# robertknight/ocrs-models

Hardware: AMD Instinct MI355X
Metric: detection train-step images/sec (higher is better)
Workload: dtype bf16

## Files before the change

### include/ocrs_hip.h

```cpp
#ifndef OCRS_HIP_H
#define OCRS_HIP_H

#ifdef __cplusplus
extern "C" {
#endif

#ifndef __HIP_PLATFORM_AMD__
typedef struct ihipStream_t* hipStream_t;
#endif

int ocrs_pack_frags(const float* src, int mode, int K, int M, int K2, long s1, long s2, long sm, void* out, int dtype, hipStream_t st);
long ocrs_pack_frags_bytes(int K, int M, int dtype);
int ocrs_pack_frags_multi(const long long* table, int n, long max_frag_threads, int dtype, hipStream_t st);

int ocrs_dwpw_fwd(const void* xa, const void* xb, int Ca, int Cb, const float* tra, const float* trb, const float* wdw, const void* wpk,
                  void* z, double* gstat, const float* gamma, void* pooled, int Cout, int N, int H, int W, int dtype, hipStream_t st);
long ocrs_dwpw_fwd_fin_supported(int Cin, int Cout, int dtype);
int ocrs_dwpw_fwd_fin(const void* xa, const void* xb, int Ca, int Cb, const float* tra, const float* trb, const float* wdw, const void* wpk, void* z,
                      double* gstat, unsigned* counter, long count, const float* bn_w, const float* bn_b, float eps, float momentum, float* tr, float* saved,
                      float* run_mean, float* run_var, long long* nbt, float lo, int Cout, int N, int H, int W, int dtype, hipStream_t st);
long ocrs_dwpw_fwd_pool_supported(int Cin, int Cout);
long ocrs_rs32_fwd_supported(int Ca, int Cb, int Cout, int dtype);
int ocrs_rs32_fwd(const float* xa, const float* xb, int Ca, int Cb, const float* tra, const float* trb, const float* wdw, const float* wpw, float* z,
                  double* gstat, const float* gamma, float* pooled, unsigned* counter, long count, const float* bn_w, const float* bn_b, float eps,
                  float momentum, float* tr, float* saved, float* run_mean, float* run_var, long long* nbt, float lo, int Cout, int N, int H, int W,
                  hipStream_t st);
long ocrs_rs32_bwd_supported(int Ca, int Cb, int Cout, int pooled, int dtype);
long ocrs_rs32_bwd_ws_floats(int Ca, int Cb, int Cout, int N, int H, int W);
int ocrs_rs32_bwd(const float* xa, const float* xb, int Ca, int Cb, const float* tra, const float* trb, const float* wdw, const float* wpw, const float* g1,
                  const float* g2, const float* z, const float* bn, const double* gsum, const float* gamma, const float* saved, float* dgamma, float* dbeta,
                  float* gxa, float* gxb, float* dwpw, float* dwdw, float* ws, const float* saved_a, double* gsum_a, const float* saved_b, double* gsum_b,
                  int pooled, int Cout, int N, int H, int W, hipStream_t st);
long ocrs_rs32_bwd_head_supported(int Ca, int Cb, int Cout, int dtype);
int ocrs_rs32_bwd_head(const float* xa, int Ca, const float* tra, const float* wdw, const float* wpw, const float* gl, const float* whead, const float* z,
                       const float* bn, const double* gsum, const float* gamma, const float* saved, float* dgamma, float* dbeta, float* gxa, float* dwpw,
                       float* dwdw, float* ws, const float* saved_a, double* gsum_a, int Cout, int N, int H, int W, hipStream_t st);
long ocrs_mm_fwd_supported(int Ca, int Cb, int Cout, int dtype);
long ocrs_mm_fwd_nparts(int Ca, int Cb, int Cout, int N, int H, int W);
int ocrs_mm_fwd(const void* xa, const void* xb, int Ca, int Cb, const float* tra, const float* trb, const float* wdw, const float* wpw, void* z,
                float* ws, const float* gamma, void* pooled, int Cout, int N, int H, int W, int dtype, hipStream_t st);
int ocrs_mm_fwd_fin(const void* xa, const void* xb, int Ca, int Cb, const float* tra, const float* trb, const float* wdw, const float* wpw, void* z, float* ws,
                    const float* gamma, void* pooled, unsigned* counter, long count, const float* bn_w, const float* bn_b, float eps, float momentum, float* tr,
                    float* saved, float* run_mean, float* run_var, long long* nbt, float lo, int Cout, int N, int H, int W, int dtype, hipStream_t st);
int ocrs_mm_fwd_fin_xu(const void* xu, const float* wexp, const float* tra, const float* wdw, const float* wpw, void* z, float* ws, unsigned* counter, long count,
                       const float* bn_w, const float* bn_b, float eps, float momentum, float* tr, float* saved, float* run_mean, float* run_var, long long* nbt,
                       float lo, int Cout, int N, int H, int W, int dtype, hipStream_t st);
int ocrs_bn_finalize_parts(const float* parts, int nparts, long count, int C, const float* gamma, const float* beta, float eps, float momentum,
                           float* tr, float* saved, float* run_mean, float* run_var, long long* nbt, float lo, hipStream_t st);
int ocrs_dwpw_c1_fwd(const float* img, const float* wdw, const float* wpw, void* z, double* gstat, int N, int H, int W, int dtype,
                     hipStream_t st);
long ocrs_dwpw_c1_u_supported(int N, int H, int W, int dtype);
int ocrs_dwpw_c1_fwd_u(const float* img, const float* wdw, const float* wpw, void* z, void* uplane, double* gstat, int N, int H, int W, int dtype,
                       hipStream_t st);
int ocrs_bn_finalize(const double* gstat, long count, int C, const float* gamma, const float* beta, float eps, float momentum, float* tr,
                     float* saved, float* run_mean, float* run_var, long long* nbt, float lo, hipStream_t st);
int ocrs_maxpool_fwd(const void* z, const float* tr, void* out, int C, int N, int H, int W, int raw, int dtype, hipStream_t st);
int ocrs_convt_fwd(const void* x, const float* tr, const void* wpk, const float* bias, void* out, int Cup, int Cout, int N, int h, int w,
                   int H, int W, int dtype, hipStream_t st);
long ocrs_rs32_convt_fwd_supported(int Cup, int Cout, int dtype);
int ocrs_rs32_convt_fwd(const float* x, const float* tr, const float* wt, const float* bias, float* out, int Cup, int Cout, int N, int h, int w, int H, int W,
                        hipStream_t st);
long ocrs_rs32_convt_dgrad_supported(int Cup, int Cout, int dtype);
int ocrs_rs32_convt_dgrad(const float* g, const float* wt, float* dx, const float* x, const float* tr, const float* saved, double* gsum, int Cup, int Cout, int N,
                          int h, int w, int H, int W, hipStream_t st);
int ocrs_head_fwd(const void* z, const float* tr, const float* w, const float* b, float* pred, long P, int dtype, hipStream_t st);

int ocrs_bn_bwd_reduce(const void* g1, const void* g2, int pooled, const void* z, const float* bn, const float* saved, double* gsum, int C,
                       int N, int H, int W, int dtype, hipStream_t st);
int ocrs_bn_bwd_finalize(const double* gsum, long count, int C, const float* gamma, const float* saved, float* coef, float* dgamma,
                         float* dbeta, hipStream_t st);
long ocrs_pw_bwd_ws_floats(int Cin, int Cout, int N, int H, int W);
int ocrs_pw_bwd(const void* xa, const void* xb, int Ca, int Cb, const float* tra, const float* trb, const float* wdw, const void* g1,
                const void* g2, int pooled, const void* z, const float* bn, const float* coef, const void* wpk_d, void* du, float* dwpw,
                float* ws, int Cout, int N, int H, int W, int dtype, hipStream_t st);
int ocrs_pw_bwd_fin(const void* xa, const void* xb, int Ca, int Cb, const float* tra, const float* trb, const float* wdw, const void* g1, const void* g2,
                    int pooled, const void* z, const float* bn, float* coef, const double* gsum, const float* gamma, const float* saved, float* dgamma,
                    float* dbeta, const void* wpk_d, void* du, float* dwpw, float* ws, int Cout, int N, int H, int W, int dtype, hipStream_t st);
long ocrs_dw_bwd_ws_floats(int C, int N, int H, int W);
int ocrs_dw_bwd(const void* xa, const void* xb, int Ca, int Cb, const float* tra, const float* trb, const float* wdw, const void* du,
                void* gxa, void* gxb, float* dwdw, float* ws, const float* saved_a, double* gsum_a, const float* saved_b, double* gsum_b,
                int N, int H, int W, int dtype, hipStream_t st);
long ocrs_mm_bwd_supported(int Ca, int Cb, int Cout, int dtype);
long ocrs_mm_bwd_ws_floats(int Ca, int Cb, int Cout, int N, int H, int W);
int ocrs_mm_bwd(const void* xa, const void* xb, int Ca, int Cb, const float* tra, const float* trb, const float* wdw, const float* wpw,
                const void* g1, const void* g2, int pooled, const void* z, const float* bn, const float* coef, void* gxa, void* gxb, float* dwpw,
                float* dwdw, float* ws, const float* saved_a, double* gsum_a, const float* saved_b, double* gsum_b, int Cout, int N, int H,
                int W, int dtype, hipStream_t st);
int ocrs_mm_bwd_fin(const void* xa, const void* xb, int Ca, int Cb, const float* tra, const float* trb, const float* wdw, const float* wpw, const void* g1,
                    const void* g2, int pooled, const void* z, const float* bn, const double* gsum, const float* gamma, const float* saved, float* dgamma,
                    float* dbeta, void* gxa, void* gxb, float* dwpw, float* dwdw, float* ws, const float* saved_a, double* gsum_a, const float* saved_b,
                    double* gsum_b, int Cout, int N, int H, int W, int dtype, hipStream_t st);
long ocrs_mm_bwd_head_supported(int Ca, int Cb, int Cout, int N, int H, int W, int dtype);
int ocrs_mm_bwd_fin_head(const void* xa, int Ca, const float* tra, const float* wdw, const float* wpw, const float* gl, const float* whead, const void* z,
                         const float* bn, const double* gsum, const float* gamma, const float* saved, float* dgamma, float* dbeta, void* gxa, float* dwpw,
                         float* dwdw, float* ws, const float* saved_a, double* gsum_a, int Cout, int N, int H, int W, int dtype, hipStream_t st);
int ocrs_mm_bwd_fin_xu(const void* xu, const float* wexp, const float* tra, const float* wdw, const float* wpw, const void* g1, const void* g2, const void* z,
                       const float* bn, const double* gsum, const float* gamma, const float* saved, float* dgamma, float* dbeta, void* gxa, float* dwpw,
                       float* dwdw, float* ws, const float* saved_a, double* gsum_a, int Cout, int N, int H, int W, int dtype, hipStream_t st);
int ocrs_dwpw_c1_bwd(const float* img, const float* wdw, const float* wpw, const void* g1, const void* g2, int pooled, const void* z,
                     const float* bn, const float* coef, double* acc64, int N, int H, int W, int dtype, hipStream_t st);
long ocrs_convt_bwd_ws_floats(int Cup, int Cout, int N, int h, int w, int dtype);
int ocrs_convt_bwd(const void* x, const float* tr, const void* g, const void* wpk_d, void* dx, float* dW, float* dbias, double* dbias64, float* ws,
// ... 213 lines not shown
```

### ocrs_models_amd/csrc/det_dwf.hip

```cpp
#include "det_common.h"

namespace {
template <int CIN, int COUT>
struct DwfCfg {
    static constexpr int NT = 512, NW = 8;
    static constexpr int TW = 8, TH = (CIN >= 128 || COUT > 128) ? 4 : 8, TP = TW * TH, NNT = TP / 16, HWp = TW + 2, HP = HWp * (TH + 2);
    static constexpr int CGI = CIN / 8;
    static constexpr int PXC = CIN + 8;
    static constexpr int NXI = (HP * CGI + NT - 1) / NT;
    static constexpr int NUI = (TP * CGI + NT - 1) / NT;
    static constexpr int MTO = COUT / 16, NKD = CIN / 32;
    static constexpr int MPW = MTO >= NW ? MTO / NW : 1;
    static constexpr int NPW = MTO >= NW ? NNT : NNT * MTO / NW;
    static constexpr int OFF_U = HP * PXC * 2, OFF_PAR = (OFF_U + TP * PXC * 2 + 15) & ~15;
    static constexpr int SMEM = OFF_PAR + (3 * CIN + 9 * CIN + NW * 2 * COUT) * 4;
    static_assert(NT % CGI == 0 && NPW >= 1 && MTO >= 4, "role mapping");
};
__device__ __forceinline__ void unpack8w(const uint4& r, float (&v)[8]) {
    v[0] = __uint_as_float(r.x << 16); v[1] = __uint_as_float(r.x & 0xffff0000u);
    v[2] = __uint_as_float(r.y << 16); v[3] = __uint_as_float(r.y & 0xffff0000u);
    v[4] = __uint_as_float(r.z << 16); v[5] = __uint_as_float(r.z & 0xffff0000u);
    v[6] = __uint_as_float(r.w << 16); v[7] = __uint_as_float(r.w & 0xffff0000u);
}
}

template <int CIN, int COUT>
__global__ __launch_bounds__(512) void k_dwf(Src2<bf16> x, const float* __restrict__ tra, const float* __restrict__ trb, const float* __restrict__ wdw,
                                             const void* __restrict__ wpk, bf16* __restrict__ z, double* __restrict__ gstat, Tiling2 tg, FwdFin fin) {
    using C = DwfCfg<CIN, COUT>;
    constexpr int NT = C::NT, TW = C::TW, TP = C::TP, HWp = C::HWp, HP = C::HP, CGI = C::CGI, PXC = C::PXC;
    constexpr int NXI = C::NXI, NUI = C::NUI, MTO = C::MTO, NKD = C::NKD, MPW = C::MPW, NPW = C::NPW;
    extern __shared__ __attribute__((aligned(16))) char smem[];
    bf16* xs = reinterpret_cast<bf16*>(smem);
    bf16* uN = reinterpret_cast<bf16*>(smem + C::OFF_U);
    float* s_trx = reinterpret_cast<float*>(smem + C::OFF_PAR);
    float* s_wdw = s_trx + 3 * CIN;
    float* s_st = s_wdw + 9 * CIN;
    const int H = tg.H, W = tg.W;
    const int tid = threadIdx.x, lane = tid & 63, wave = __builtin_amdgcn_readfirstlane(tid >> 6);
    fill_tr8(s_trx, x, tra, trb, CIN, tid);
    for (int i = tid; i < 9 * CIN; i += NT) {
        const int t = i / CIN, c = i - t * CIN;
        s_wdw[i] = wdw[c * 9 + t];
    }
    {
        const uint4 z4 = make_uint4(0, 0, 0, 0);
        for (int i = tid; i < C::OFF_PAR / 16; i += NT) reinterpret_cast<uint4*>(smem)[i] = z4;
    }
    __syncthreads();

    const int cgi = tid % CGI;
    const int m0w = MTO >= C::NW ? wave * MPW : wave % MTO, n0w = MTO >= C::NW ? 0 : (wave / MTO) * NPW;
    Mma<bf16>::Frag wf[NKD][MPW];
#pragma unroll
    for (int kc = 0; kc < NKD; ++kc)
#pragma unroll
        for (int a = 0; a < MPW; ++a) wf[kc][a] = Mma<bf16>::load_w(wpk, (long)kc * MTO + m0w + a, lane);
    float s1[MPW][4], s2[MPW][4];
#pragma unroll
    for (int a = 0; a < MPW; ++a)
#pragma unroll
        for (int i = 0; i < 4; ++i) s1[a][i] = s2[a][i] = 0.f;

    struct Raw {
        uint4 xr[NXI];
        unsigned okx;
    };
    auto issue = [&](Raw& r, const TileOrg& org) {
        r.okx = 0;
        const int c0 = cgi * 8;
        const bool from_a = c0 < x.Ca;
        const bf16* xb = from_a ? x.a + c0 : x.b + (c0 - x.Ca);
        const int pitch = from_a ? x.Ca : x.Cb;
        const long corner = ((long)org.n * H + (org.h0 - 1)) * W + (org.w0 - 1);
#pragma unroll
        for (int j = 0; j < NXI; ++j) {
            const int hp = (tid + j * NT) / CGI, hy = hp / HWp, hx = hp - hy * HWp;
            const int h = org.h0 - 1 + hy, w = org.w0 - 1 + hx;
            const bool ok = (HP * CGI % NT == 0 || tid + j * NT < HP * CGI) && (unsigned)h < (unsigned)H && (unsigned)w < (unsigned)W;
            r.xr[j] = *reinterpret_cast<const uint4*>(ok ? xb + (corner + (long)hy * W + hx) * pitch : xb);
            r.okx |= ok ? 1u << j : 0u;
        }
    };
    auto commit = [&](const Raw& r) {
        float sc[8], sh[8], lo[8];
        load8(s_trx + cgi * 24, sc);
        load8(s_trx + cgi * 24 + 8, sh);
        load8(s_trx + cgi * 24 + 16, lo);
#pragma unroll
        for (int j = 0; j < NXI; ++j) {
            if (HP * CGI % NT != 0 && tid + j * NT >= HP * CGI) break;
            float v[8] = {0.f, 0.f, 0.f, 0.f, 0.f, 0.f, 0.f, 0.f};
            if (r.okx & (1u << j)) {
                unpack8w(r.xr[j], v);
#pragma unroll
                for (int i = 0; i < 8; ++i) v[i] = max_lo(fmaf(v[i], sc[i], sh[i]), lo[i]);
            }
            store8_opaque(xs + ((tid + j * NT) / CGI) * PXC + cgi * 8, v);
            __builtin_amdgcn_sched_barrier(0);
        }
    };

    TileSched ts(tg.ntiles);
    Raw cur;
    if (ts.first < ts.end) issue(cur, tile_origin2<TW, C::TH>(tg, (int)ts.first));
    for (long t = ts.first; t < ts.end; t += ts.step) {
        const TileOrg org = tile_origin2<TW, C::TH>(tg, (int)t);
        commit(cur);
        __syncthreads();
        if (t + ts.step < ts.end) issue(cur, tile_origin2<TW, C::TH>(tg, (int)(t + ts.step)));
        {
            float u[NUI][8];
#pragma unroll
            for (int j = 0; j < NUI; ++j)
#pragma unroll
                for (int i = 0; i < 8; ++i) u[j][i] = 0.f;
#pragma unroll
            for (int tap = 0; tap < 9; ++tap) {
                float wv[8];
                load8(s_wdw + tap * CIN + cgi * 8, wv);
#pragma unroll
                for (int j = 0; j < NUI; ++j) {
                    const int pxl = (tid + j * NT) / CGI, ty = pxl / TW, tx = pxl - ty * TW;
                    if (TP * CGI % NT == 0 || tid + j * NT < TP * CGI) {
                        float v[8];
                        unpack8w(*reinterpret_cast<const uint4*>(xs + ((ty + tap / 3) * HWp + tx + tap % 3) * PXC + cgi * 8), v);
#pragma unroll
                        for (int i = 0; i < 8; ++i) u[j][i] = fmaf(wv[i], v[i], u[j][i]);
                    }
                }
                if (tap % 3 == 2) __builtin_amdgcn_sched_barrier(0);
            }
#pragma unroll
            for (int j = 0; j < NUI; ++j)
                if (TP * CGI % NT == 0 || tid + j * NT < TP * CGI) store8_opaque(uN + ((tid + j * NT) / CGI) * PXC + cgi * 8, u[j]);
        }
        __syncthreads();
        {
            f32x4 acc[MPW][NPW];
#pragma unroll
            for (int a = 0; a < MPW; ++a)
#pragma unroll
                for (int b = 0; b < NPW; ++b) acc[a][b] = (f32x4){0.f, 0.f, 0.f, 0.f};
#pragma unroll
            for (int kc = 0; kc < NKD; ++kc)
#pragma unroll
                for (int b = 0; b < NPW; ++b) {
                    const Mma<bf16>::Frag pf = Mma<bf16>::load_p(uN + kc * 32, PXC, (n0w + b) * 16, lane, 32);
#pragma unroll
                    for (int a = 0; a < MPW; ++a) acc[a][b] = Mma<bf16>::template mma<8>(wf[kc][a], pf, acc[a][b]);
                }
#pragma unroll
            for (int b = 0; b < NPW; ++b) {
                const int oq = (n0w + b) * 16 + (lane & 15);
                const int qh = org.h0 + oq / TW, qw = org.w0 + oq % TW;
                if (qh < H && qw < W) {
                    bf16* dst = z + (((long)org.n * H + qh) * W + qw) * COUT + m0w * 16 + (lane >> 4) * 4;
#pragma unroll
                    for (int a = 0; a < MPW; ++a) {
                        const f32x4 v = acc[a][b];
                        store4(dst + a * 16, v[0], v[1], v[2], v[3]);
#pragma unroll
                        for (int i = 0; i < 4; ++i) {
                            const float q = Elem<bf16>::round(v[i]);
                            s1[a][i] += q;
                            s2[a][i] = fmaf(q, q, s2[a][i]);
                        }
                    }
                }
            }
        }
    }
    for (int i = tid; i < C::NW * 2 * COUT; i += NT) s_st[i] = 0.f;
    __syncthreads();
#pragma unroll
    for (int a = 0; a < MPW; ++a)
#pragma unroll
        for (int i = 0; i < 4; ++i) {
            const float v1 = quad16_sum(s1[a][i]), v2 = quad16_sum(s2[a][i]);
            if ((lane & 15) == 0) {
                const int m = (m0w + a) * 16 + (lane >> 4) * 4 + i;
                s_st[(wave * 2 + 0) * COUT + m] = v1;
                s_st[(wave * 2 + 1) * COUT + m] = v2;
            }
        }
    __syncthreads();
    for (int i = tid; i < 2 * COUT; i += NT) {
        const int which = i / COUT, m = i - which * COUT;
        float s = 0.f;
        for (int w = 0; w < C::NW; ++w) s += s_st[(w * 2 + which) * COUT + m];
        atomicAdd(&gstat[i], (double)s);
    }
    bn_finalize_last_block(fin, gstat, COUT, tid, NT, reinterpret_cast<int*>(smem));
}

extern "C" {

long det_dwf_supported(int Cin, int Cout, int dtype) {
    return dtype == 1 && (Cin == 32 || Cin == 64 || Cin == 128 || Cin == 256) && (Cout == 64 || Cout == 128 || Cout == 256) && Cin * 8 >= Cout;
}

int det_dwf_launch(const void* xa, const void* xb, int Ca, int Cb, const float* tra, const float* trb, const float* wdw, const void* wpk, void* z,
                   double* gstat, int Cout, int N, int H, int W, hipStream_t st, const FwdFin& fin) {
    const int Cin = Ca + Cb;
    OCRS_CHECK_ARG(det_dwf_supported(Cin, Cout, 1) && Ca % 8 == 0 && Cb % 8 == 0);
    Src2<bf16> x{(const bf16*)xa, (const bf16*)xb, Ca, Cb};
    bool done = false;
#define DWF_CASE(CI_, CO_)                                                                                                                   \
    if (!done && Cin == CI_ && Cout == CO_) {                                                                                                \
        using CC = DwfCfg<CI_, CO_>;                                                                                                         \
        static DevOnce attr_set;                                                                                                        \
        if (attr_set.need()) {                                                                                                                     \
            if (hipFuncSetAttribute(reinterpret_cast<const void*>(&k_dwf<CI_, CO_>), hipFuncAttributeMaxDynamicSharedMemorySize, CC::SMEM) != \
                hipSuccess)                                                                                                                  \
                return OCRS_ERR_HIP;                                                                                                         \
            attr_set.done();                                                                                                                 \
        }                                                                                                                                    \
        const Tiling2 tg = make_tiling2(N, H, W, CC::TW, CC::TH);                                                                            \
        long g = tg.ntiles;                                                                                                                  \
        const long cap = (long)kNumCU * (CI_ <= 128 ? 2 : 1);                                                                 \
        if (g > cap) g = cap;                                                                                                                \
        if (g >= 8) g &= ~7L;                                                                                                                \
        hipLaunchKernelGGL((k_dwf<CI_, CO_>), dim3((int)g), dim3(512), CC::SMEM, st, x, tra, trb, wdw, wpk, (bf16*)z, gstat, tg, fin);       \
        done = true;                                                                                                                         \
    }
    DWF_CASE(32, 64) DWF_CASE(64, 64) DWF_CASE(64, 128) DWF_CASE(128, 64) DWF_CASE(128, 128) DWF_CASE(128, 256) DWF_CASE(256, 128) DWF_CASE(256, 256)
#undef DWF_CASE
    OCRS_CHECK_ARG(done);
    OCRS_LAUNCH_CHECK();
    return OCRS_OK;
}

}
```

### ocrs_models_amd/csrc/det_fwd.hip

```cpp
#include "det_common.h"

template <class T>
__device__ __forceinline__ void pack_frags_body(const float* __restrict__ src, int mode, int K, int M, int K2, long s1, long s2, long sm, T* __restrict__ out,
                                                long idx) {
    const int MT = (M + 15) / 16;
    const int nkc = (K + 31) / 32;
    if (idx >= (long)nkc * MT * 64) return;
    const int lane = (int)(idx & 63);
    const long frag = idx >> 6;
    const int mt = (int)(frag % MT), kc = (int)(frag / MT);
    const int m = mt * 16 + (lane & 15);
    float v[8];
#pragma unroll
    for (int j = 0; j < 8; ++j) {
        const int k = Elem<T>::is_bf16 ? kc * 32 + (lane >> 4) * 8 + j : kc * 32 + j * 4 + (lane >> 4);
        float x = 0.f;
        if (k < K && m < M) {
            if (mode == 0 || mode == 2) {
                x = src[(long)(k / K2) * s1 + (long)(k % K2) * s2 + (long)m * sm];
            } else {
                const int Cup = K2, Cout = M / 4;
                const int d = k / Cup, c = k % Cup, q = m / Cout, o = m % Cout;
                const int ky = (q >> 1) + 2 * (d >> 1), kx = (q & 1) + 2 * (d & 1);
                if (ky < 3 && kx < 3) x = src[((long)c * Cout + o) * 9 + ky * 3 + kx];
// ... 393 lines not shown
        pred[p] = 1.f / (1.f + __expf(-s));
    }
}

static inline int ew_grid(long items) {
    long g = (items + 255) / 256;
    const long cap = (long)kNumCU * 8;
    return (int)(g < 1 ? 1 : (g > cap ? cap : g));
}

extern "C" {

int ocrs_pack_frags(const float* src, int mode, int K, int M, int K2, long s1, long s2, long sm, void* out, int dtype, hipStream_t st) {
    OCRS_CHECK_ARG(src && out && K > 0 && M > 0 && K2 > 0);
    const long n = (long)((K + 31) / 32) * ((M + 15) / 16) * 64;
    const int grid = (int)((n + 255) / 256);
    if (dtype == 1)
        hipLaunchKernelGGL(k_pack_frags<bf16>, dim3(grid), dim3(256), 0, st, src, mode, K, M, K2, s1, s2, sm, (bf16*)out);
    else
        hipLaunchKernelGGL(k_pack_frags<float>, dim3(grid), dim3(256), 0, st, src, mode, K, M, K2, s1, s2, sm, (float*)out);
    OCRS_LAUNCH_CHECK();
    return OCRS_OK;
}

int ocrs_pack_frags_multi(const long long* table, int n, long max_frag_threads, int dtype, hipStream_t st) {
    OCRS_CHECK_ARG(table && n > 0 && max_frag_threads > 0);
    const dim3 grid((unsigned)((max_frag_threads + 255) / 256), (unsigned)n);
    if (dtype == 1)
        hipLaunchKernelGGL(k_pack_frags_multi<bf16>, grid, dim3(256), 0, st, table);
    else
        hipLaunchKernelGGL(k_pack_frags_multi<float>, grid, dim3(256), 0, st, table);
    OCRS_LAUNCH_CHECK();
    return OCRS_OK;
}

long ocrs_pack_frags_bytes(int K, int M, int dtype) { return (long)((K + 31) / 32) * ((M + 15) / 16) * 64 * 8 * (dtype == 1 ? 2 : 4); }

}
template <class T, int CG, int MT, bool ONE>
static int launch_dwpw_fwd(const void* xa, const void* xb, int Ca, int Cb, const float* tra, const float* trb, const float* wdw, const void* wpk, void* z,
                           double* gstat, int COUT, int N, int H, int W, const float* gamma, void* pooled, hipStream_t st) {
    using FT = FwdTile<CG, FwdPx<MT>::PX>;
    constexpr int TP = FT::TP;
    const int CIN = Ca + Cb;
    Src2<T> x{(const T*)xa, (const T*)xb, Ca, Cb};
    const Tiling2 tg = make_tiling2(N, H, W, FT::TW, FT::TH);
    const size_t smem = ((TP * FwdPitch<T, CG>::V * sizeof(T) + 15) & ~15) +
                        (HaloTile<FT::TW, FT::TH>::HP * CG * 8 + 12 * CIN + 4 * 2 * MT * 16) * sizeof(float);
    const int tpb = tg.ntiles >= 2048 ? 2 : 1;
    const int grid = persistent_grid(tg.ntiles / tpb > 0 ? tg.ntiles / tpb : 1, 4);
    if (pooled) {
        if constexpr (FwdPx<MT>::PX == 2 && FT::TW >= 16)
            hipLaunchKernelGGL((k_dwpw_fwd<T, CG, MT, ONE, true>), dim3(grid), dim3(256), smem, st, x, tra, trb, wdw, wpk, (T*)z, gstat, CIN, COUT, tg,
                               gamma, (T*)pooled);
        else
            return OCRS_ERR_ARG;
    } else
        hipLaunchKernelGGL((k_dwpw_fwd<T, CG, MT, ONE, false>), dim3(grid), dim3(256), smem, st, x, tra, trb, wdw, wpk, (T*)z, gstat, CIN, COUT, tg,
                           gamma, (T*)pooled);
    OCRS_LAUNCH_CHECK();
    return OCRS_OK;
}
extern "C" {

}

template <class T>
static int dispatch_dwpw_fwd(const void* xa, const void* xb, int Ca, int Cb, const float* tra, const float* trb, const float* wdw, const void* wpk, void* z,
                             double* gstat, int COUT, int N, int H, int W, const float* gamma, void* pooled, hipStream_t st) {
    const int CIN = Ca + Cb;
    const int cg = CIN >= 32 ? 4 : CIN / 8;
    const int mt = (COUT + 15) / 16;
#define DWPW_CASE(CG_, MT_, ONE_) \
    if (cg == CG_ && mt == MT_ && (CIN == CG_ * 8) == ONE_) \
        return launch_dwpw_fwd<T, CG_, MT_, ONE_>(xa, xb, Ca, Cb, tra, trb, wdw, wpk, z, gstat, COUT, N, H, W, gamma, pooled, st);
    DWPW_CASE(1, 1, true) DWPW_CASE(2, 1, true) DWPW_CASE(2, 2, true)
    DWPW_CASE(4, 1, true) DWPW_CASE(4, 2, true) DWPW_CASE(4, 4, true)
    DWPW_CASE(4, 1, false) DWPW_CASE(4, 2, false) DWPW_CASE(4, 4, false) DWPW_CASE(4, 8, false) DWPW_CASE(4, 16, false)
#undef DWPW_CASE
    return OCRS_ERR_ARG;
}
extern "C" {

long det_dwf_supported(int Cin, int Cout, int dtype);
long det_c1v2_supported(int N, int H, int W);
int det_c1v2_fwd_launch(const float* img, const float* wdw, const float* wpw, void* z, double* gstat, int N, int H, int W, int dtype, hipStream_t st,
                        void* uplane, double* fsum);
int det_c1_bwd_fin_launch(const double* c1acc, const double* fsum, const float* coef, const float* wexp, double* acc64, hipStream_t st);
int det_dwf_launch(const void* xa, const void* xb, int Ca, int Cb, const float* tra, const float* trb, const float* wdw, const void* wpk, void* z,
                   double* gstat, int Cout, int N, int H, int W, hipStream_t st, const FwdFin& fin);
long ocrs_dwpw_fwd_pool_supported(int Cin, int Cout) {
    if (det_dwf_supported(Cin, Cout, 1)) return 0;
    return Cout <= 64 && (Cin < 32 || Cin % 32 == 0) ? 1 : 0;
}

int ocrs_dwpw_fwd(const void* xa, const void* xb, int Ca, int Cb, const float* tra, const float* trb, const float* wdw, const void* wpk,
                  void* z, double* gstat, const float* gamma, void* pooled, int Cout, int N, int H, int W, int dtype, hipStream_t st) {
    const int Cin = Ca + Cb;
    OCRS_CHECK_ARG(!pooled || (gamma && ocrs_dwpw_fwd_pool_supported(Cin, Cout)));
    OCRS_CHECK_ARG(xa && tra && wdw && wpk && z && gstat && (Cb == 0 || trb));
    OCRS_CHECK_ARG(Ca % 8 == 0 && Cb % 8 == 0 && Cin >= 8 && (Cin < 32 || Cin % 32 == 0) && Cout % 8 == 0 && Cout <= 256);
    OCRS_CHECK_ARG((Cb == 0) == (xb == nullptr));
    OCRS_CHECK_ARG((long)N * H * W < (1L << 31));
    if (!pooled && det_dwf_supported(Cin, Cout, dtype))
        return det_dwf_launch(xa, xb, Ca, Cb, tra, trb, wdw, wpk, z, gstat, Cout, N, H, W, st, FwdFin{nullptr, 0, nullptr, nullptr, 0.f, 0.f, nullptr, nullptr, nullptr, nullptr, nullptr, 0.f});
    return dtype == 1 ? dispatch_dwpw_fwd<bf16>(xa, xb, Ca, Cb, tra, trb, wdw, wpk, z, gstat, Cout, N, H, W, gamma, pooled, st)
                      : dispatch_dwpw_fwd<float>(xa, xb, Ca, Cb, tra, trb, wdw, wpk, z, gstat, Cout, N, H, W, gamma, pooled, st);
}

long ocrs_dwpw_fwd_fin_supported(int Cin, int Cout, int dtype) { return det_dwf_supported(Cin, Cout, dtype); }
int ocrs_dwpw_fwd_fin(const void* xa, const void* xb, int Ca, int Cb, const float* tra, const float* trb, const float* wdw, const void* wpk, void* z,
                      double* gstat, unsigned* counter, long count, const float* bn_w, const float* bn_b, float eps, float momentum, float* tr, float* saved,
                      float* run_mean, float* run_var, long long* nbt, float lo, int Cout, int N, int H, int W, int dtype, hipStream_t st) {
    const int Cin = Ca + Cb;
    OCRS_CHECK_ARG(xa && tra && wdw && wpk && z && gstat && (Cb == 0 || trb) && (Cb == 0) == (xb == nullptr));
    OCRS_CHECK_ARG(counter && count > 0 && bn_w && bn_b && tr && saved && ocrs_dwpw_fwd_fin_supported(Cin, Cout, dtype) && (long)N * H * W < (1L << 31));
    return det_dwf_launch(xa, xb, Ca, Cb, tra, trb, wdw, wpk, z, gstat, Cout, N, H, W, st,
                          FwdFin{counter, count, bn_w, bn_b, eps, momentum, tr, saved, run_mean, run_var, nbt, lo});
}

int ocrs_dwpw_c1_fwd(const float* img, const float* wdw, const float* wpw, void* z, double* gstat, int N, int H, int W, int dtype,
                     hipStream_t st) {
    OCRS_CHECK_ARG(img && wdw && wpw && z && gstat);
    if (det_c1v2_supported(N, H, W)) return det_c1v2_fwd_launch(img, wdw, wpw, z, gstat, N, H, W, dtype, st, nullptr, nullptr);
    const long P = (long)N * H * W;
    const int grid = ew_grid(P);
    if (dtype == 1)
        hipLaunchKernelGGL(k_dwpw_c1_fwd<bf16>, dim3(grid), dim3(256), 0, st, img, wdw, wpw, (bf16*)z, gstat, H, W, P);
    else
        hipLaunchKernelGGL(k_dwpw_c1_fwd<float>, dim3(grid), dim3(256), 0, st, img, wdw, wpw, (float*)z, gstat, H, W, P);
    OCRS_LAUNCH_CHECK();
    return OCRS_OK;
}

long ocrs_dwpw_c1_u_supported(int N, int H, int W, int dtype) { return dtype == 1 && det_c1v2_supported(N, H, W) ? 1 : 0; }
int ocrs_dwpw_c1_fwd_u(const float* img, const float* wdw, const float* wpw, void* z, void* uplane, double* gstat, int N, int H, int W, int dtype,
                       hipStream_t st) {
    OCRS_CHECK_ARG(img && wdw && wpw && uplane && gstat && ocrs_dwpw_c1_u_supported(N, H, W, dtype));
    return det_c1v2_fwd_launch(img, wdw, wpw, z, gstat, N, H, W, dtype, st, uplane, nullptr);
}
int ocrs_dwpw_c1_fwd_us(const float* img, const float* wdw, const float* wpw, void* z, void* uplane, double* gstat, double* fsum, int N, int H, int W, int dtype,
                        hipStream_t st) {
    OCRS_CHECK_ARG(img && wdw && wpw && uplane && gstat && fsum && dtype == 1 && ocrs_dwpw_c1_u_supported(N, H, W, dtype));
    return det_c1v2_fwd_launch(img, wdw, wpw, z, gstat, N, H, W, dtype, st, uplane, fsum);
}
int ocrs_c1_bwd_fin(const double* c1acc, const double* fsum, const float* coef, const float* wexp, double* acc64, hipStream_t st) {
    OCRS_CHECK_ARG(c1acc && fsum && coef && wexp && acc64);
    return det_c1_bwd_fin_launch(c1acc, fsum, coef, wexp, acc64, st);
}

int ocrs_bn_finalize(const double* gstat, long count, int C, const float* gamma, const float* beta, float eps, float momentum, float* tr,
                     float* saved, float* run_mean, float* run_var, long long* nbt, float lo, hipStream_t st) {
    OCRS_CHECK_ARG(gstat && gamma && beta && tr && saved && C > 0 && count > 0);
    hipLaunchKernelGGL(k_bn_finalize, dim3((C + 63) / 64), dim3(64), 0, st, gstat, count, C, gamma, beta, eps, momentum, tr, saved, run_mean,
                       run_var, nbt, lo);
    OCRS_LAUNCH_CHECK();
    return OCRS_OK;
}

int ocrs_maxpool_fwd(const void* z, const float* tr, void* out, int C, int N, int H, int W, int raw, int dtype, hipStream_t st) {
    OCRS_CHECK_ARG(z && tr && out && C % 8 == 0 && H >= 2 && W >= 2 && (raw == 0 || raw == 1));
    const long Pp = (long)N * (H / 2) * (W / 2);
    const int grid = ew_grid(Pp * (C / 8));
#define OCRS_POOL(T_, R_) hipLaunchKernelGGL((k_maxpool_fwd<T_, R_>), dim3(grid), dim3(256), 0, st, (const T_*)z, tr, (T_*)out, C, H, W, Pp)
    if (dtype == 1) {
        if (raw) OCRS_POOL(bf16, true);
        else OCRS_POOL(bf16, false);
    } else {
        if (raw) OCRS_POOL(float, true);
        else OCRS_POOL(float, false);
    }
#undef OCRS_POOL
    OCRS_LAUNCH_CHECK();
    return OCRS_OK;
}

}
template <int CUP, int COUT>
struct CtfCfg {
    static constexpr int TH = 8, TW = 16, TPOS = TH * TW;
    static constexpr int XH = TH + 1, XW = TW + 1, XP = XH * XW;
    static constexpr int NKC = 4 * CUP / 32, MT = 4 * COUT / 16;
    static constexpr int XI = XP * CUP / 8, NXI = (XI + 255) / 256;
    static constexpr int XPITCH = CUP + 8;
    static constexpr int SMEM = (XP * XPITCH + NKC * MT * 64 * 8) * 2 + 3 * CUP * 4 + 4 * COUT * 4;
};
template <int CUP, int COUT>
__global__ __launch_bounds__(256) void k_convt_fwd_tile(const bf16* __restrict__ x, const float* __restrict__ tr, const void* __restrict__ wpk,
                                                        const float* __restrict__ bias, bf16* __restrict__ out, int h, int w, int H, int W,
                                                        Tiling2 tg) {
    using C = CtfCfg<CUP, COUT>;
    constexpr int TW = C::TW, TH = C::TH, XW = C::XW, MT = C::MT, NKC = C::NKC, XPITCH = C::XPITCH;
    extern __shared__ __attribute__((aligned(16))) char smem[];
    bf16* xs = reinterpret_cast<bf16*>(smem);
    uint4* s_wf = reinterpret_cast<uint4*>(xs + C::XP * XPITCH);
    float* s_tr = reinterpret_cast<float*>(s_wf + NKC * MT * 64);
    float* s_bias = s_tr + 3 * CUP;
    const int tid = threadIdx.x, lane = tid & 63, wave = tid >> 6;
    {
        Src2<bf16> xsrc{x, nullptr, CUP, 0};
        fill_tr8(s_tr, xsrc, tr, nullptr, CUP, tid);
// ... 156 lines not shown
```

### ocrs_models_amd/models.py

```python
from __future__ import annotations

import math

import torch
from torch import nn

from ._lib import lib, ptr
from .packs import EMPTY as EMPTY_PACKS, PackRow, cached_table, dgrad_row, fwd_row

DEPTH_SCALE = [8, 16, 32, 32, 64, 128, 256]
_DT = {torch.float32: 0, torch.bfloat16: 1}


class DepthwiseConv(nn.Module):

    def __init__(self, in_channels: int, out_channels: int):
        super().__init__()
        self.seq = nn.Sequential(
            nn.Conv2d(in_channels, in_channels, 3, padding=1, bias=False, groups=in_channels),
            nn.Conv2d(in_channels, out_channels, 1, bias=False),
            nn.BatchNorm2d(out_channels),
            nn.ReLU(),
        )

# ... 149 lines not shown
        for i in range(6):
            rows += [self.convt_row(P[f"up.{i}.up.weight"]), self.convt_dgrad_row(P[f"up.{i}.up.weight"])]
        return rows

    def prepack(self):
        key = (self.dt, tuple(p.data_ptr() for p in self.P.values()))
        self.packs = cached_table(self.mod, key, self.pack_rows, self.dev)
        self.packs.launch()

    def bn_tr(self, prefix, gstat, count, C, nparts=0):
        P, Bf = self.P, self.Bf
        tr, saved, fin = self.bn_fin(prefix, C)
        if self.train and nparts:
            self.L.bn_finalize_parts(ptr(gstat), nparts, count, C, *fin)
        elif self.train:
            self.L.bn_finalize(ptr(gstat), count, C, *fin)
        else:
            rstd = torch.rsqrt(Bf[f"{prefix}.running_var"] + 1e-5)
            tr[0] = P[f"{prefix}.weight"].detach() * rstd
            tr[1] = P[f"{prefix}.bias"].detach() - Bf[f"{prefix}.running_mean"] * tr[0]
            tr[2] = 0.0
        return tr, saved

    def fwd_route(self, Ca, Cb, Cout, H, W):
        if self.use_mm and self.L.mm_fwd_supported(Ca, Cb, Cout, self.dt):
            return "mm"
        if self.use_rs32 and self.L.rs32_fwd_supported(Ca, Cb, Cout, self.dt) and self.fits32(H, W, max(Ca + Cb, Cout)):
            return "rs32"
        return "tile"

    def bwd_route(self, r, pooled, need_gx):
        if r.Cin == 1:
            return "c1"
        L, C, H, W = self.L, r.Cout, r.H, r.W
        Ca, Cb = r.a.C, (r.b.C if r.b is not None else 0)
        if self.use_mm and need_gx and H >= 2 and W >= 2 and L.mm_bwd_supported(Ca, Cb, C, self.dt):
            return "mm"
        if (self.use_rs32 and need_gx and L.rs32_bwd_supported(Ca, Cb, C, 1 if pooled else 0, self.dt) and self.fits32(H, W, max(r.Cin, C))
                and (not pooled or (H >= 2 and W >= 2))):
            return "rs32"
        return "tile"

    def block(self, prefix, a, b, Cout, pool=False):
        L, P, N = self.L, self.P, self.N
        H, W = a.H, a.W
        Cb = b.C if b is not None else 0
        Cin = a.C + Cb
        wdw, wpw = P[f"{prefix}.seq.0.weight"], P[f"{prefix}.seq.1.weight"]
        z = self.empty(N, H, W, Cout)
        bnp = f"{prefix}.seq.2"
        fin = self.train and self.fold_fwd_fin
        pooled = gamma = None
        route = self.fwd_route(a.C, Cb, Cout, H, W)
        if route == "mm":
            if pool:
                pooled, gamma = self.empty(N, H // 2, W // 2, Cout), P[f"{bnp}.weight"]
            nparts = L.mm_fwd_nparts(a.C, Cb, Cout, N, H, W)
            parts = self.empty(nparts * 2 * Cout, dtype=torch.float32)
            if fin and a.u is not None and b is None and pooled is None and Cout in (8, 16):
                tr, saved, fin_args = self.bn_fin(bnp, Cout)
                L.mm_fwd_fin_xu(ptr(a.u), ptr(a.wexp), ptr(a.tr), ptr(wdw), ptr(wpw), ptr(z), ptr(parts), ptr(self.zeros64(1)), N * H * W, *fin_args,
                                Cout, N, H, W, self.dt)
            elif fin:
                tr, saved, fin_args = self.bn_fin(bnp, Cout)
                L.mm_fwd_fin(*_srcs(a, b), ptr(wdw), ptr(wpw), ptr(z), ptr(parts), ptr(gamma), ptr(pooled), ptr(self.zeros64(1)), N * H * W, *fin_args,
                             Cout, N, H, W, self.dt)
            else:
                L.mm_fwd(*_srcs(a, b), ptr(wdw), ptr(wpw), ptr(z), ptr(parts), ptr(gamma), ptr(pooled), Cout, N, H, W, self.dt)
                tr, saved = self.bn_tr(bnp, parts, N * H * W, Cout, nparts=nparts)
        elif route == "rs32":
            if pool:
                pooled, gamma = self.empty(N, H // 2, W // 2, Cout), P[f"{bnp}.weight"]
            gstat = self.zeros64(2 * Cout)
            common = (*_srcs(a, b), ptr(wdw), ptr(wpw), ptr(z), ptr(gstat), ptr(gamma), ptr(pooled))
            if fin:
                tr, saved, fin_args = self.bn_fin(bnp, Cout)
                L.rs32_fwd(*common, ptr(self.zeros64(1)), N * H * W, *fin_args, Cout, N, H, W)
            else:
                L.rs32_fwd(*common, None, 0, None, None, 0.0, 0.0, None, None, None, None, None, 0.0, Cout, N, H, W)
                tr, saved = self.bn_tr(bnp, gstat, N * H * W, Cout)
        else:
            wpk = self.packs.fetch(fwd_row(wpw, self.dt), self.dev)
            gstat = self.zeros64(2 * Cout)
            if pool and L.dwpw_fwd_pool_supported(Cin, Cout):
                pooled, gamma = self.empty(N, H // 2, W // 2, Cout), P[f"{bnp}.weight"]
            if fin and pooled is None and L.dwpw_fwd_fin_supported(Cin, Cout, self.dt):
                tr, saved, fin_args = self.bn_fin(bnp, Cout)
                L.dwpw_fwd_fin(*_srcs(a, b), ptr(wdw), ptr(wpk), ptr(z), ptr(gstat), ptr(self.zeros64(1)), N * H * W, *fin_args, Cout, N, H, W, self.dt)
            else:
                L.dwpw_fwd(*_srcs(a, b), ptr(wdw), ptr(wpk), ptr(z), ptr(gstat), ptr(gamma), ptr(pooled), Cout, N, H, W, self.dt)
                tr, saved = self.bn_tr(bnp, gstat, N * H * W, Cout)
        self.pooled_by_block = pooled
        self.recs[prefix] = _BlockRec(prefix, a, b, z, tr, saved, Cin, Cout, H, W)
        return _Act(z, tr, Cout, H, W, src=prefix)

    def block_c1(self, prefix, img, H, W):
        L, P, N = self.L, self.P, self.N
        wdw, wpw = P[f"{prefix}.seq.0.weight"], P[f"{prefix}.seq.1.weight"]
        z = self.empty(N, H, W, 8)
        gstat = self.zeros64(16)
        uplane = fsum = None
        if self.train and self.c1_u and self.use_mm and L.dwpw_c1_u_supported(N, H, W, self.dt):
            uplane = torch.empty(N, H, W, dtype=torch.bfloat16, device=self.dev)
            if (self.c1_noz and self.capture is None and self.fold_fwd_fin and self.fuse_bn_bwd and L.mm_fwd_supported(8, 0, 8, self.dt)
                    and L.mm_bwd_head_supported(8, 0, 8, N, H, W, self.dt)):
                z = None
            fsum = self.zeros64(20) if (z is None and self.c1_fuse) else None
            if fsum is not None:
                L.dwpw_c1_fwd_us(ptr(img), ptr(wdw), ptr(wpw), ptr(z), ptr(uplane), ptr(gstat), ptr(fsum), N, H, W, self.dt)
            else:
                L.dwpw_c1_fwd_u(ptr(img), ptr(wdw), ptr(wpw), ptr(z), ptr(uplane), ptr(gstat), N, H, W, self.dt)
        else:
            L.dwpw_c1_fwd(ptr(img), ptr(wdw), ptr(wpw), ptr(z), ptr(gstat), N, H, W, self.dt)
        tr, saved = self.bn_tr(f"{prefix}.seq.2", gstat, N * H * W, 8)
        self.recs[prefix] = _BlockRec(prefix, None, None, z, tr, saved, 1, 8, H, W, fsum)
        out = _Act(z, tr, 8, H, W, src=prefix)
        out.u, out.wexp = uplane, wpw
        return out

    def double(self, prefix, a, b, Cout, pool=False):
        y = self.block(f"{prefix}.seq.0", a, b, Cout)
        return self.block(f"{prefix}.seq.1", y, None, Cout, pool=pool)

    def forward(self):
        L, P, N, w = self.L, self.P, self.N, DEPTH_SCALE
        x = self.x
        H, W = x.shape[2], x.shape[3]
        if H < 64 or W < 64:
            raise RuntimeError(f"DetectionModel needs H, W >= 64 (six 2x2 poolings), got {H}x{W}")
        self.prepack()
        a0 = self.block_c1("in_conv.seq.0", x, H, W)
        cur = self.block("in_conv.seq.1", a0, None, w[0])
        skips = [cur]
        for i in range(6):
            y = self.double(f"down.{i}.seq.0", cur, None, w[i + 1], pool=True)
            Hp, Wp = y.H // 2, y.W // 2
            pooled = self.pooled_by_block
            y.other_use = True
            if pooled is None:
                pooled = self.empty(N, Hp, Wp, y.C)
                L.maxpool_fwd(ptr(y.t), ptr(y.tr), ptr(pooled), y.C, N, y.H, y.W, 1, self.dt)
            cur = _Act(pooled, y.tr, y.C, Hp, Wp, src=y.src)
            skips.append(cur)
        up = skips[6]
        self.convt = {}
        for i in reversed(range(6)):
            skip = skips[i]
            Cup, Cout = w[i + 1], w[i]
            wpk = self.packs.fetch(self.convt_row(P[f"up.{i}.up.weight"]), self.dev)
            t = self.empty(N, skip.H, skip.W, Cout)
            up.other_use = True
            if self.use_rs32 and L.rs32_convt_fwd_supported(Cup, Cout, self.dt) and self.fits32(skip.H, skip.W, Cout):
                L.rs32_convt_fwd(ptr(up.t), ptr(up.tr), ptr(P[f"up.{i}.up.weight"]), ptr(P[f"up.{i}.up.bias"]), ptr(t), Cup, Cout, N, up.H, up.W, skip.H, skip.W)
            else:
                L.convt_fwd(ptr(up.t), ptr(up.tr), ptr(wpk), ptr(P[f"up.{i}.up.bias"]), ptr(t), Cup, Cout, N, up.H, up.W, skip.H, skip.W, self.dt)
            ta = _Act(t, _identity_tr(Cout, self.dev), Cout, skip.H, skip.W)
            self.convt[i] = (up, ta)
            up = self.double(f"up.{i}.contract", ta, skip, Cout)
        pred = self.empty(N, 1, H, W, dtype=torch.float32)
        up.other_use = True
        L.head_fwd(ptr(up.t), ptr(up.tr), ptr(P["out_conv.0.weight"]), ptr(P["out_conv.0.bias"]), ptr(pred), N * H * W, self.dt)
        self.head_in, self.pred, self.skips, self.HW = up, pred, skips, (H, W)
        return pred

    def block_bwd(self, prefix, g1, g2, pooled, need_gx=True):
        gxa, gxb = self._block_bwd(prefix, g1, g2, pooled, need_gx)
        if self.capture is not None:
            self.capture[prefix] = {"g1": g1, "g2": g2, "pooled": pooled, "gxa": gxa, "gxb": gxb}
        return gxa, gxb

    def _block_bwd(self, prefix, g1, g2, pooled, need_gx=True):
# ... 334 lines not shown
```

Measured before the change: 2768.

## Fuse 2x2 max-pool into deep dwf forward kernel and double-buffer tile loads

Adds a fused 2x2 max-pool epilogue to the bf16 depthwise+pointwise forward kernel, using DPP lane shuffles and a gamma-sign flip so the pool stays correct after the later BN affine. Deep blocks that pool can now use the fast dwf/fin path instead of the generic fallback. The kernel also gets two register sets for prefetching input tiles on some channel configs, plus occupancy launch bounds. The extra prefetch registers and launch-bound limits may cause spills.

```diff
diff --git a/include/ocrs_hip.h b/include/ocrs_hip.h
--- a/include/ocrs_hip.h
+++ b/include/ocrs_hip.h
@@ -17,7 +17,7 @@
                   void* z, double* gstat, const float* gamma, void* pooled, int Cout, int N, int H, int W, int dtype, hipStream_t st);
 long ocrs_dwpw_fwd_fin_supported(int Cin, int Cout, int dtype);
 int ocrs_dwpw_fwd_fin(const void* xa, const void* xb, int Ca, int Cb, const float* tra, const float* trb, const float* wdw, const void* wpk, void* z,
-                      double* gstat, unsigned* counter, long count, const float* bn_w, const float* bn_b, float eps, float momentum, float* tr, float* saved,
+                      double* gstat, const float* gamma, void* pooled, unsigned* counter, long count, const float* bn_w, const float* bn_b, float eps, float momentum, float* tr, float* saved,
                       float* run_mean, float* run_var, long long* nbt, float lo, int Cout, int N, int H, int W, int dtype, hipStream_t st);
 long ocrs_dwpw_fwd_pool_supported(int Cin, int Cout);
 long ocrs_rs32_fwd_supported(int Ca, int Cb, int Cout, int dtype);
diff --git a/ocrs_models_amd/csrc/det_dwf.hip b/ocrs_models_amd/csrc/det_dwf.hip
--- a/ocrs_models_amd/csrc/det_dwf.hip
+++ b/ocrs_models_amd/csrc/det_dwf.hip
@@ -14,6 +14,8 @@
     static constexpr int NPW = MTO >= NW ? NNT : NNT * MTO / NW;
     static constexpr int OFF_U = HP * PXC * 2, OFF_PAR = (OFF_U + TP * PXC * 2 + 15) & ~15;
     static constexpr int SMEM = OFF_PAR + (3 * CIN + 9 * CIN + NW * 2 * COUT) * 4;
+    static constexpr int SETS = ((CIN == 64 || CIN == 128) && COUT <= 128) ? 2 : 1;
+    static constexpr bool POOL = !(CIN == 128 && COUT == 256);
     static_assert(NT % CGI == 0 && NPW >= 1 && MTO >= 4, "role mapping");
 };
 __device__ __forceinline__ void unpack8w(const uint4& r, float (&v)[8]) {
@@ -22,11 +24,21 @@
     v[4] = __uint_as_float(r.z << 16); v[5] = __uint_as_float(r.z & 0xffff0000u);
     v[6] = __uint_as_float(r.w << 16); v[7] = __uint_as_float(r.w & 0xffff0000u);
 }
+template <int MPW>
+__device__ __forceinline__ unsigned pool_neg_mask(const float* __restrict__ gamma, int m) {
+    unsigned mask = 0;
+#pragma unroll
+    for (int a = 0; a < MPW; ++a)
+#pragma unroll
+        for (int i = 0; i < 4; ++i) mask |= gamma[m + a * 16 + i] < 0.f ? 1u << (a * 4 + i) : 0u;
+    return mask;
+}
 }
 
 template <int CIN, int COUT>
-__global__ __launch_bounds__(512) void k_dwf(Src2<bf16> x, const float* __restrict__ tra, const float* __restrict__ trb, const float* __restrict__ wdw,
-                                             const void* __restrict__ wpk, bf16* __restrict__ z, double* __restrict__ gstat, Tiling2 tg, FwdFin fin) {
+__global__ __launch_bounds__(512, (CIN <= 128 ? 4 : 2)) void k_dwf(Src2<bf16> x, const float* __restrict__ tra, const float* __restrict__ trb, const float* __restrict__ wdw,
+                                             const void* __restrict__ wpk, bf16* __restrict__ z, double* __restrict__ gstat, Tiling2 tg, FwdFin fin,
+                                             const float* __restrict__ gamma, bf16* __restrict__ pooled ) {
     using C = DwfCfg<CIN, COUT>;
     constexpr int NT = C::NT, TW = C::TW, TP = C::TP, HWp = C::HWp, HP = C::HP, CGI = C::CGI, PXC = C::PXC;
     constexpr int NXI = C::NXI, NUI = C::NUI, MTO = C::MTO, NKD = C::NKD, MPW = C::MPW, NPW = C::NPW;
@@ -66,7 +78,7 @@
         uint4 xr[NXI];
         unsigned okx;
     };
-    auto issue = [&](Raw& r, const TileOrg& org) {
+    auto issue = [&](Raw& r, const TileOrg& org, bool live) __attribute__((always_inline)) {
         r.okx = 0;
         const int c0 = cgi * 8;
         const bool from_a = c0 < x.Ca;
@@ -77,12 +89,12 @@
         for (int j = 0; j < NXI; ++j) {
             const int hp = (tid + j * NT) / CGI, hy = hp / HWp, hx = hp - hy * HWp;
             const int h = org.h0 - 1 + hy, w = org.w0 - 1 + hx;
-            const bool ok = (HP * CGI % NT == 0 || tid + j * NT < HP * CGI) && (unsigned)h < (unsigned)H && (unsigned)w < (unsigned)W;
+            const bool ok = live && (HP * CGI % NT == 0 || tid + j * NT < HP * CGI) && (unsigned)h < (unsigned)H && (unsigned)w < (unsigned)W;
             r.xr[j] = *reinterpret_cast<const uint4*>(ok ? xb + (corner + (long)hy * W + hx) * pitch : xb);
             r.okx |= ok ? 1u << j : 0u;
         }
     };
-    auto commit = [&](const Raw& r) {
+    auto commit = [&](const Raw& r) __attribute__((always_inline)) {
         float sc[8], sh[8], lo[8];
         load8(s_trx + cgi * 24, sc);
         load8(s_trx + cgi * 24 + 8, sh);
@@ -101,14 +113,18 @@
         }
     };
 
+    constexpr int SETS = C::SETS;
     TileSched ts(tg.ntiles);
-    Raw cur;
-    if (ts.first < ts.end) issue(cur, tile_origin2<TW, C::TH>(tg, (int)ts.first));
-    for (long t = ts.first; t < ts.end; t += ts.step) {
+    const unsigned negm = (C::POOL && pooled) ? pool_neg_mask<MPW>(gamma, m0w * 16 + (lane >> 4) * 4) : 0u;
+    auto issue_at = [&](Raw& r, long t) __attribute__((always_inline)) {
+        const bool live = t < ts.end;
+        issue(r, tile_origin2<TW, C::TH>(tg, live ? (int)t : 0), live);
+    };
+    auto tile = [&](Raw& r, long t) __attribute__((always_inline)) {
         const TileOrg org = tile_origin2<TW, C::TH>(tg, (int)t);
-        commit(cur);
+        commit(r);
         __syncthreads();
-        if (t + ts.step < ts.end) issue(cur, tile_origin2<TW, C::TH>(tg, (int)(t + ts.step)));
+        if (SETS == 2 || t + ts.step < ts.end) issue_at(r, t + SETS * ts.step);
         {
             float u[NUI][8];
 #pragma unroll
@@ -169,6 +185,41 @@
                     }
                 }
             }
+            if (C::POOL && pooled) {
+#pragma unroll
+              for (int b = 0; b < NPW; ++b) {
+                const int oq = (n0w + b) * 16 + (lane & 15);
+                const int Hp = H >> 1, Wp = W >> 1, ph = (org.h0 + oq / TW) >> 1, pw = (org.w0 + oq % TW) >> 1;
+                const bool owner = (lane & 9) == 0 && ph < Hp && pw < Wp;
+                bf16* dst = pooled + (((long)org.n * Hp + ph) * Wp + pw) * COUT + m0w * 16 + (lane >> 4) * 4;
+#pragma unroll
+                for (int a = 0; a < MPW; ++a) {
+                    float m4[4];
+#pragma unroll
+                    for (int i = 0; i < 4; ++i) {
+                        const unsigned flip = ((negm >> (a * 4 + i)) & 1u) << 31;
+                        float k = __uint_as_float(__float_as_uint(Elem<bf16>::round(acc[a][b][i])) ^ flip);
+                        const float right = dpp_f<0xB1>(k);
+                        k = right > k ? right : k;
+                        const float below = dpp_f<0x128>(k);
+                        k = below > k ? below : k;
+                        m4[i] = __uint_as_float(__float_as_uint(k) ^ flip);
+                    }
+                    if (owner) store4(dst + a * 16, m4[0], m4[1], m4[2], m4[3]);
+                }
+              }
+            }
+        }
+    };
+    Raw ra;
+    [[maybe_unused]] Raw rb;
+    issue_at(ra, ts.first);
+    if constexpr (SETS == 2) issue_at(rb, ts.first + ts.step);
+    for (long t = ts.first; t < ts.end; t += SETS * ts.step) {
+        tile(ra, t);
+        if constexpr (SETS == 2) {
+            if (t + ts.step >= ts.end) break;
+            tile(rb, t + ts.step);
         }
     }
     for (int i = tid; i < C::NW * 2 * COUT; i += NT) s_st[i] = 0.f;
@@ -199,11 +250,12 @@
 long det_dwf_supported(int Cin, int Cout, int dtype) {
     return dtype == 1 && (Cin == 32 || Cin == 64 || Cin == 128 || Cin == 256) && (Cout == 64 || Cout == 128 || Cout == 256) && Cin * 8 >= Cout;
 }
+long det_dwf_pool_supported(int Cin, int Cout) { return det_dwf_supported(Cin, Cout, 1) && !(Cin == 128 && Cout == 256); }
 
 int det_dwf_launch(const void* xa, const void* xb, int Ca, int Cb, const float* tra, const float* trb, const float* wdw, const void* wpk, void* z,
-                   double* gstat, int Cout, int N, int H, int W, hipStream_t st, const FwdFin& fin) {
+                   double* gstat, int Cout, int N, int H, int W, hipStream_t st, const FwdFin& fin, const float* gamma, void* pooled) {
     const int Cin = Ca + Cb;
-    OCRS_CHECK_ARG(det_dwf_supported(Cin, Cout, 1) && Ca % 8 == 0 && Cb % 8 == 0);
+    OCRS_CHECK_ARG(det_dwf_supported(Cin, Cout, 1) && Ca % 8 == 0 && Cb % 8 == 0 && (!pooled || (gamma && det_dwf_pool_supported(Cin, Cout))));
     Src2<bf16> x{(const bf16*)xa, (const bf16*)xb, Ca, Cb};
     bool done = false;
 #define DWF_CASE(CI_, CO_)                                                                                                                   \
@@ -221,7 +273,8 @@
         const long cap = (long)kNumCU * (CI_ <= 128 ? 2 : 1);                                                                 \
         if (g > cap) g = cap;                                                                                                                \
         if (g >= 8) g &= ~7L;                                                                                                                \
-        hipLaunchKernelGGL((k_dwf<CI_, CO_>), dim3((int)g), dim3(512), CC::SMEM, st, x, tra, trb, wdw, wpk, (bf16*)z, gstat, tg, fin);       \
+        hipLaunchKernelGGL((k_dwf<CI_, CO_>), dim3((int)g), dim3(512), CC::SMEM, st, x, tra, trb, wdw, wpk, (bf16*)z, gstat, tg, fin, \
+                           gamma, (bf16*)pooled);                                                                                            \
         done = true;                                                                                                                         \
     }
     DWF_CASE(32, 64) DWF_CASE(64, 64) DWF_CASE(64, 128) DWF_CASE(128, 64) DWF_CASE(128, 128) DWF_CASE(128, 256) DWF_CASE(256, 128) DWF_CASE(256, 256)
diff --git a/ocrs_models_amd/csrc/det_fwd.hip b/ocrs_models_amd/csrc/det_fwd.hip
--- a/ocrs_models_amd/csrc/det_fwd.hip
+++ b/ocrs_models_amd/csrc/det_fwd.hip
@@ -499,15 +499,16 @@
 }
 extern "C" {
 
+long det_dwf_pool_supported(int Cin, int Cout);
 long det_dwf_supported(int Cin, int Cout, int dtype);
 long det_c1v2_supported(int N, int H, int W);
 int det_c1v2_fwd_launch(const float* img, const float* wdw, const float* wpw, void* z, double* gstat, int N, int H, int W, int dtype, hipStream_t st,
                         void* uplane, double* fsum);
 int det_c1_bwd_fin_launch(const double* c1acc, const double* fsum, const float* coef, const float* wexp, double* acc64, hipStream_t st);
 int det_dwf_launch(const void* xa, const void* xb, int Ca, int Cb, const float* tra, const float* trb, const float* wdw, const void* wpk, void* z,
-                   double* gstat, int Cout, int N, int H, int W, hipStream_t st, const FwdFin& fin);
+                   double* gstat, int Cout, int N, int H, int W, hipStream_t st, const FwdFin& fin, const float* gamma, void* pooled);
 long ocrs_dwpw_fwd_pool_supported(int Cin, int Cout) {
-    if (det_dwf_supported(Cin, Cout, 1)) return 0;
+    if (det_dwf_supported(Cin, Cout, 1)) return det_dwf_pool_supported(Cin, Cout);
     return Cout <= 64 && (Cin < 32 || Cin % 32 == 0) ? 1 : 0;
 }
 
@@ -519,21 +520,23 @@
     OCRS_CHECK_ARG(Ca % 8 == 0 && Cb % 8 == 0 && Cin >= 8 && (Cin < 32 || Cin % 32 == 0) && Cout % 8 == 0 && Cout <= 256);
     OCRS_CHECK_ARG((Cb == 0) == (xb == nullptr));
     OCRS_CHECK_ARG((long)N * H * W < (1L << 31));
-    if (!pooled && det_dwf_supported(Cin, Cout, dtype))
-        return det_dwf_launch(xa, xb, Ca, Cb, tra, trb, wdw, wpk, z, gstat, Cout, N, H, W, st, FwdFin{nullptr, 0, nullptr, nullptr, 0.f, 0.f, nullptr, nullptr, nullptr, nullptr, nullptr, 0.f});
+    if (det_dwf_supported(Cin, Cout, dtype))
+        return det_dwf_launch(xa, xb, Ca, Cb, tra, trb, wdw, wpk, z, gstat, Cout, N, H, W, st,
+                              FwdFin{nullptr, 0, nullptr, nullptr, 0.f, 0.f, nullptr, nullptr, nullptr, nullptr, nullptr, 0.f}, gamma, pooled);
     return dtype == 1 ? dispatch_dwpw_fwd<bf16>(xa, xb, Ca, Cb, tra, trb, wdw, wpk, z, gstat, Cout, N, H, W, gamma, pooled, st)
                       : dispatch_dwpw_fwd<float>(xa, xb, Ca, Cb, tra, trb, wdw, wpk, z, gstat, Cout, N, H, W, gamma, pooled, st);
 }
 
 long ocrs_dwpw_fwd_fin_supported(int Cin, int Cout, int dtype) { return det_dwf_supported(Cin, Cout, dtype); }
 int ocrs_dwpw_fwd_fin(const void* xa, const void* xb, int Ca, int Cb, const float* tra, const float* trb, const float* wdw, const void* wpk, void* z,
-                      double* gstat, unsigned* counter, long count, const float* bn_w, const float* bn_b, float eps, float momentum, float* tr, float* saved,
+                      double* gstat, const float* gamma, void* pooled, unsigned* counter, long count, const float* bn_w, const float* bn_b, float eps, float momentum, float* tr, float* saved,
                       float* run_mean, float* run_var, long long* nbt, float lo, int Cout, int N, int H, int W, int dtype, hipStream_t st) {
     const int Cin = Ca + Cb;
     OCRS_CHECK_ARG(xa && tra && wdw && wpk && z && gstat && (Cb == 0 || trb) && (Cb == 0) == (xb == nullptr));
     OCRS_CHECK_ARG(counter && count > 0 && bn_w && bn_b && tr && saved && ocrs_dwpw_fwd_fin_supported(Cin, Cout, dtype) && (long)N * H * W < (1L << 31));
+    OCRS_CHECK_ARG(!pooled || gamma);
     return det_dwf_launch(xa, xb, Ca, Cb, tra, trb, wdw, wpk, z, gstat, Cout, N, H, W, st,
-                          FwdFin{counter, count, bn_w, bn_b, eps, momentum, tr, saved, run_mean, run_var, nbt, lo});
+                          FwdFin{counter, count, bn_w, bn_b, eps, momentum, tr, saved, run_mean, run_var, nbt, lo}, gamma, pooled);
 }
 
 int ocrs_dwpw_c1_fwd(const float* img, const float* wdw, const float* wpw, void* z, double* gstat, int N, int H, int W, int dtype,
diff --git a/ocrs_models_amd/models.py b/ocrs_models_amd/models.py
--- a/ocrs_models_amd/models.py
+++ b/ocrs_models_amd/models.py
@@ -255,11 +255,13 @@
         else:
             wpk = self.packs.fetch(fwd_row(wpw, self.dt), self.dev)
             gstat = self.zeros64(2 * Cout)
-            if pool and L.dwpw_fwd_pool_supported(Cin, Cout):
+            deep = L.dwpw_fwd_fin_supported(Cin, Cout, self.dt)
+            if pool and L.dwpw_fwd_pool_supported(Cin, Cout) and (deep or not L.dwpw_fwd_fin_supported(Cin, Cout, 1)):
                 pooled, gamma = self.empty(N, H // 2, W // 2, Cout), P[f"{bnp}.weight"]
-            if fin and pooled is None and L.dwpw_fwd_fin_supported(Cin, Cout, self.dt):
+            if fin and deep:
                 tr, saved, fin_args = self.bn_fin(bnp, Cout)
-                L.dwpw_fwd_fin(*_srcs(a, b), ptr(wdw), ptr(wpk), ptr(z), ptr(gstat), ptr(self.zeros64(1)), N * H * W, *fin_args, Cout, N, H, W, self.dt)
+                L.dwpw_fwd_fin(*_srcs(a, b), ptr(wdw), ptr(wpk), ptr(z), ptr(gstat), ptr(gamma), ptr(pooled), ptr(self.zeros64(1)), N * H * W, *fin_args,
+                               Cout, N, H, W, self.dt)
             else:
                 L.dwpw_fwd(*_srcs(a, b), ptr(wdw), ptr(wpk), ptr(z), ptr(gstat), ptr(gamma), ptr(pooled), Cout, N, H, W, self.dt)
                 tr, saved = self.bn_tr(bnp, gstat, N * H * W, Cout)
```

Result: slower. 2719 (-1.8%).
